# sahaRatul/sela

Hardware: AMD Instinct MI355X
Metric: Msamples/s encode+decode, 16-bit stereo 44.1kHz, 1/2/4/8 GPU; bit-exact vs CPU (higher is better)
Workload: dtype f64+int64

## Files before the change

### include/sela_hip_debug.h

```cpp
#ifndef SELA_HIP_DEBUG_H_
#define SELA_HIP_DEBUG_H_

#include <stddef.h>
#include <stdint.h>

#ifdef __cplusplus
extern "C" {
#endif

void sela_hip_debug_phase_buffer(uint64_t* d_cycles);
void sela_hip_debug_force_plain_fir(int enable);
void sela_hip_debug_mean_workers(int self_blocks);
void sela_hip_debug_encode_teams(int lanes);
int sela_hip_debug_encode_kernel(uint32_t n_frames, uint32_t channels);
void sela_hip_debug_encode_fused(int enable);
void sela_hip_debug_priorities(uint32_t team_quarters);
void sela_hip_debug_priorities_adaptive(void);
int sela_hip_debug_launches_alone(void);
void sela_hip_debug_keep_both_candidates(int on);
void sela_hip_debug_stage_wait(int naps);
int sela_hip_debug_reissued_feeds(void);
void sela_hip_debug_decode_recurrence(int form);
int sela_hip_debug_contexts_created(void);
void sela_hip_debug_coalesced(int kind, long long* batches, long long* retried);
size_t sela_hip_debug_verify_lds_bytes(uint32_t channels);
size_t sela_hip_debug_levels_lds_bytes(uint32_t channels);
size_t sela_hip_debug_digest_lds_bytes(uint32_t channels);
long long sela_hip_debug_verify_i32_fallback_frames(const void* d_workspace, uint32_t max_frames, uint32_t channels, uint32_t stride);
long long sela_hip_debug_verify_pcm_fallback_frames(const void* d_workspace, uint32_t max_frames, uint32_t channels, uint32_t stride);
long long sela_hip_debug_levels_i32_fallback_frames(const void* d_workspace, uint32_t max_frames, uint32_t channels, uint32_t stride);
long long sela_hip_debug_digest_pcm_fallback_frames(const void* d_workspace, uint32_t max_frames, uint32_t channels, uint32_t stride);

void sela_hip_debug_encode_hashes(int on);
int sela_hip_debug_block_forms(const void* d_workspace, uint32_t n_frames, uint32_t channels, uint32_t* counts_out, uint8_t* forms_out);
void sela_hip_debug_encode_split(int mode);
int sela_hip_debug_launches_split(void);
void sela_hip_debug_standard_first(int mode);
int sela_hip_debug_standard_chunks(void);
long long sela_hip_debug_segment_subframes(void);
void sela_hip_debug_generic_wrap_taps(int on);
size_t sela_hip_debug_window_lds_bytes(uint32_t channels);
uint64_t sela_hip_debug_windows_staged_bytes(void);
enum {
    SELA_HIP_WORKSPACE_ENCODE = 0, SELA_HIP_WORKSPACE_DECODE, SELA_HIP_WORKSPACE_INDEX, SELA_HIP_WORKSPACE_DECODE_I32, SELA_HIP_WORKSPACE_DECODE_N,
    SELA_HIP_WORKSPACE_VERIFY, SELA_HIP_WORKSPACE_VERIFY_I32, SELA_HIP_WORKSPACE_ENCODE_I32, SELA_HIP_WORKSPACE_ENCODE_PAIRED, SELA_HIP_WORKSPACE_WINDOWS,
// ... 11 lines not shown
```

### sela_amd/capi.py

```python
from __future__ import annotations

import ctypes as C
import os

HERE = os.path.dirname(os.path.abspath(__file__))
LIB_PATH = os.path.join(HERE, "libsela_hip.so")

OK = 0
ERRORS = {-1: "ENODEV", -2: "EINVAL", -3: "ENOMEM", -4: "ECAPACITY", -5: "EFORMAT", -6: "ERANGE"}
SAMPLES_PER_FRAME = 2048

FLAG_Q_RANGE, FLAG_COEF_OVERFLOW, FLAG_RICE_RANGE, FLAG_RICE_OVERRUN, FLAG_WORDS_CAP, FLAG_BAD_FRAME, FLAG_INTERNAL, FLAG_SHORT_BLOCK = 1, 2, 4, 8, 16, 32, 64, 128
FLAG_STRIDE = 256

EXPORTS = [
    "sela_hip_init", "sela_hip_shutdown", "sela_hip_thread_release", "sela_hip_last_error", "sela_hip_device_count",
    "sela_hip_signals_per_frame", "sela_hip_encode_workspace_bytes", "sela_hip_decode_workspace_bytes",
    "sela_hip_encode_bound_bytes", "sela_hip_encode_device", "sela_hip_decode_device",
    "sela_hip_encode", "sela_hip_decode", "sela_hip_index_frames",
    "sela_hip_enable_kernel_timing", "sela_hip_kernel_times",
    "sela_hip_lpc_encode", "sela_hip_lpc_decode", "sela_hip_rice_encode", "sela_hip_rice_decode",
    "sela_hip_host_alloc", "sela_hip_host_free", "sela_hip_decode_max_channels",
    "sela_hip_encode_begin", "sela_hip_encode_feed", "sela_hip_encode_end",
    "sela_hip_decode_begin", "sela_hip_decode_feed", "sela_hip_decode_end",
# ... 22 lines not shown
    "sela_hip_encode_pcm_device", "sela_hip_decode_pcm_workspace_bytes", "sela_hip_decode_pcm_device", "sela_hip_decode_pcm_status_error",
    "sela_hip_encode_pcm", "sela_hip_decode_pcm",
    "sela_hip_verify_pcm_workspace_bytes", "sela_hip_verify_pcm_device", "sela_hip_verify_payload_pcm_device", "sela_hip_verify_pcm",
    "sela_hip_levels_workspace_bytes", "sela_hip_levels_device", "sela_hip_levels_payload_device", "sela_hip_levels",
    "sela_hip_levels_i32_workspace_bytes", "sela_hip_levels_i32_device", "sela_hip_levels_payload_i32_device", "sela_hip_levels_samples_i32_workspace_bytes",
    "sela_hip_levels_samples_i32_device", "sela_hip_levels_i32",
    "sela_hip_digest_workspace_bytes", "sela_hip_digest_device", "sela_hip_digest_payload_device", "sela_hip_digest", "sela_hip_crc32_combine",
    "sela_hip_crc32_workspace_bytes", "sela_hip_crc32_device",
    "sela_hip_digest_pcm_workspace_bytes", "sela_hip_digest_pcm_device", "sela_hip_digest_payload_pcm_device", "sela_hip_digest_pcm",
    "sela_hip_salvage_frames", "sela_hip_salvage_workspace_bytes", "sela_hip_salvage_frames_device", "sela_hip_salvage_payload_device",
]
WINDOW_I16_INTERLEAVED, WINDOW_F32_PLANAR = 0, 1
WINDOW_I32_PLANAR, WINDOW_PCM24_INTERLEAVED, WINDOW_PCM32_INTERLEAVED = 2, 3, 4
ENCODE_LOSSLESS = 1



DEBUG_EXPORTS = [
    "sela_hip_debug_phase_buffer", "sela_hip_debug_force_plain_fir", "sela_hip_debug_mean_workers", "sela_hip_debug_encode_teams", "sela_hip_debug_encode_kernel", "sela_hip_debug_encode_fused", "sela_hip_debug_priorities", "sela_hip_debug_priorities_adaptive", "sela_hip_debug_launches_alone", "sela_hip_debug_block_forms", "sela_hip_debug_encode_hashes", "sela_hip_debug_standard_first", "sela_hip_debug_standard_chunks", "sela_hip_debug_segment_subframes", "sela_hip_debug_generic_wrap_taps", "sela_hip_debug_encode_split", "sela_hip_debug_launches_split", "sela_hip_debug_keep_both_candidates", "sela_hip_debug_stage_wait",
    "sela_hip_debug_reissued_feeds", "sela_hip_debug_contexts_created", "sela_hip_debug_decode_recurrence", "sela_hip_debug_coalesced", "sela_hip_debug_verify_lds_bytes",
    "sela_hip_debug_verify_i32_fallback_frames", "sela_hip_debug_window_lds_bytes", "sela_hip_debug_windows_staged_bytes",
    "sela_hip_debug_workspace_pieces", "sela_hip_debug_pcm_chunk_frames", "sela_hip_debug_verify_pcm_fallback_frames",
    "sela_hip_debug_levels_lds_bytes", "sela_hip_debug_levels_i32_fallback_frames", "sela_hip_debug_digest_lds_bytes",
    "sela_hip_debug_digest_pcm_fallback_frames",
]
WORKSPACE_CALLS = ("encode", "decode", "index", "decode_i32", "decode_n", "verify", "verify_i32", "encode_i32", "encode_paired", "windows", "windows_whole",
                   "encode_whole", "encode_split", "decode_whole", "windows_i32", "windows_i32_whole", "encode_whole_pcm", "salvage")


class Trace(C.Structure):
    _fields_ = [
        ("mean", C.c_double), ("ac", C.c_double * 101), ("k", C.c_double * 100), ("a", C.c_int64 * 101),
        ("q", C.c_int32 * 100), ("order", C.c_int32), ("coef_k", C.c_uint32), ("coef_words", C.c_uint32),
        ("res_k", C.c_uint32), ("res_words", C.c_uint32), ("flags", C.c_uint32),
    ]


class SelaHipError(RuntimeError):
    def __init__(self, code: int, message: str):
        super().__init__(f"libsela_hip: {ERRORS.get(code, code)}: {message}")
        self.code = code


_LIB = None


def lib() -> C.CDLL:
# ... 274 lines not shown
    L.sela_hip_debug_standard_first.restype = None
    L.sela_hip_debug_standard_chunks.argtypes = []
    L.sela_hip_debug_standard_chunks.restype = C.c_int
    L.sela_hip_debug_segment_subframes.argtypes = []
    L.sela_hip_debug_segment_subframes.restype = C.c_longlong
    L.sela_hip_debug_generic_wrap_taps.argtypes = [C.c_int]
    L.sela_hip_debug_generic_wrap_taps.restype = None
    L.sela_hip_debug_encode_split.argtypes = [C.c_int]
    L.sela_hip_debug_encode_split.restype = None
    L.sela_hip_debug_launches_split.argtypes = []
    L.sela_hip_debug_launches_split.restype = C.c_int
    L.sela_hip_debug_block_forms.argtypes = [C.c_void_p, C.c_uint32, C.c_uint32, C.c_void_p, C.c_void_p]
    L.sela_hip_debug_block_forms.restype = C.c_int
    L.sela_hip_debug_keep_both_candidates.argtypes = [C.c_int]
    L.sela_hip_debug_keep_both_candidates.restype = None
    L.sela_hip_debug_encode_kernel.argtypes = [C.c_uint32, C.c_uint32]
    L.sela_hip_debug_encode_kernel.restype = C.c_int
    L.sela_hip_debug_stage_wait.argtypes = [C.c_int]
    L.sela_hip_debug_stage_wait.restype = None
    L.sela_hip_debug_reissued_feeds.argtypes = []
    L.sela_hip_debug_reissued_feeds.restype = C.c_int
    L.sela_hip_debug_decode_recurrence.argtypes = [C.c_int]
    L.sela_hip_debug_decode_recurrence.restype = None
    L.sela_hip_debug_contexts_created.argtypes = []
    L.sela_hip_debug_contexts_created.restype = C.c_int
    L.sela_hip_debug_coalesced.argtypes = [C.c_int, C.POINTER(C.c_longlong), C.POINTER(C.c_longlong)]
    L.sela_hip_debug_coalesced.restype = None
    L.sela_hip_debug_verify_lds_bytes.argtypes = [u32]
    L.sela_hip_debug_verify_lds_bytes.restype = sz
    L.sela_hip_debug_verify_i32_fallback_frames.argtypes = [vp, u32, u32, u32]
    L.sela_hip_debug_verify_pcm_fallback_frames.argtypes = [vp, u32, u32, u32]
    L.sela_hip_debug_verify_pcm_fallback_frames.restype = C.c_longlong
    L.sela_hip_debug_verify_i32_fallback_frames.restype = C.c_longlong
    L.sela_hip_debug_window_lds_bytes.argtypes = [u32]
    L.sela_hip_debug_window_lds_bytes.restype = sz
    L.sela_hip_debug_windows_staged_bytes.argtypes = []
    L.sela_hip_debug_windows_staged_bytes.restype = C.c_uint64
    L.sela_hip_debug_workspace_pieces.argtypes = [C.c_int, u64, u32, u32, u64p, C.c_int]
    L.sela_hip_debug_workspace_pieces.restype = C.c_int
    L.sela_hip_host_alloc.argtypes = [sz]
    L.sela_hip_host_alloc.restype = C.c_void_p
    L.sela_hip_host_free.argtypes = [C.c_void_p]
    L.sela_hip_host_free.restype = None
    L.sela_hip_decode_max_channels.argtypes = []
    L.sela_hip_decode_max_channels.restype = u32
    L.sela_hip_encode_begin.argtypes = [C.POINTER(C.c_void_p), u32, u32, vp, sz, vp]
# ... 32 lines not shown
```

### sela_amd/csrc/sela_capi.hip

```cpp
#include <hip/hip_runtime.h>

#include <algorithm>
#include <atomic>

#include <chrono>
#include <condition_variable>
#include <deque>
#include <thread>
#include <cstdio>
#include <cstdlib>
#include <cstring>
#include <map>
#include <mutex>
#include <string>
#include <vector>

#include "sela_coalescer.h"
#include "sela_crc32.h"
#include "sela_decode_whole_plan.h"
#include "sela_host.h"
#include "sela_lease.h"
#include "sela_pcm.h"
#include "sela_salvage_walk.h"

// ... 53 lines not shown
    for (const Verdict& v : table)
        if ((flags & v.flag) && (v.routes & route))
            return fail(v.code, v.named ? std::string(who) + ": " + v.text : std::string(v.text));
    return SELA_HIP_OK;
}

}
namespace sela {
int report_error(int code, const std::string& what) { return fail(code, what); }
int report_hip_error(hipError_t e, const char* where) { return fail_hip(e, where); }
int device_ready()
{
    int n = 0;
    if (hipGetDeviceCount(&n) != hipSuccess || n <= 0)
        return fail(SELA_HIP_ENODEV, "no HIP device visible (the SELA MI355X path has no CPU fallback)");
    return SELA_HIP_OK;
}
int check_frame_offsets(const uint64_t* frame_offsets, uint32_t n_frames)
{
    return frame_offsets_ascend(frame_offsets, n_frames) ? SELA_HIP_OK : fail(SELA_HIP_EFORMAT, "frame offsets must not decrease");
}
int judge_decode(uint32_t flags, uint32_t judged, DecodeRoute route, const char* who) { return judge(kDecodeVerdicts, flags & judged, 1u << route, who); }
int judge_encode(uint32_t flags, uint32_t judged, const char* who) { return judge(kEncodeVerdicts, flags & judged, kEveryRoute, who); }
}
namespace {

struct PinnedPool {
    struct Block {
        void* ptr;
        size_t cap;
        bool pinned;
    };
    std::mutex mu;
    std::vector<Block> live, idle;
    size_t idle_bytes = 0;
    static constexpr size_t kIdleCap = (size_t)1 << 30;

    void* take(size_t bytes)
    {
        std::lock_guard<std::mutex> lock(mu);
        size_t best = idle.size();
        for (size_t i = 0; i < idle.size(); i++)
            if (idle[i].cap >= bytes && idle[i].cap <= 2 * bytes + 4096 && (best == idle.size() || idle[i].cap < idle[best].cap))
                best = i;
        Block b;
        if (best != idle.size()) {
// ... 1060 lines not shown
        }
    }
    if (e != hipSuccess)
        return fail_hip(e, "block forms");
    for (size_t b = 0; b < blocks; b++) {
        const uint32_t form = (meta[b].flags & sela::kBlockFormPlain) ? 2 : ((meta[b].flags & sela::kBlockFormTwoPass) ? 1 : 0);
        counts_out[form]++;
        if (forms_out)
            forms_out[b] = (uint8_t)form;
    }
    return SELA_HIP_OK;
}
void sela_hip_debug_keep_both_candidates(int on) { sela::set_keep_both_candidates(on); }
void sela_hip_debug_encode_split(int mode) { g_encode_split.store(mode < 0 || mode > 999 ? 0 : mode, std::memory_order_relaxed); }
int sela_hip_debug_launches_split(void) { return g_launches_split.load(std::memory_order_relaxed); }
void sela_hip_debug_encode_hashes(int on) { sela::set_encode_hashes(on); }
int sela_hip_debug_encode_kernel(uint32_t n_frames, uint32_t channels) { return sela::encode_team_lanes(n_frames, channels, g_team_lanes); }

void sela_hip_debug_stage_wait(int naps) { g_stage_wait_naps = naps; }

int sela_hip_debug_reissued_feeds(void) { return g_reissued_feeds; }
void sela_hip_debug_decode_recurrence(int form) { g_recurrence_form = form < 0 ? -1 : (form != 0); }
int sela_hip_debug_contexts_created(void) { return g_contexts_created.load(std::memory_order_relaxed); }

void sela_hip_enable_kernel_timing(int enable) { g_timing.enabled = enable != 0; }

int sela_hip_kernel_times(float* ms_out, int capacity)
{
    const int n = g_timing.recorded < capacity ? g_timing.recorded : capacity;
    for (int i = 0; i < n; i++) {
        if (hipEventSynchronize(g_timing.ev[i + 1]) != hipSuccess || hipEventElapsedTime(&ms_out[i], g_timing.ev[i], g_timing.ev[i + 1]) != hipSuccess)
            return 0;
    }
    return n;
}

uint32_t sela_hip_signals_per_frame(uint32_t channels) { return channels == 2 ? 3u : channels; }

size_t sela_hip_encode_workspace_bytes(uint32_t n_frames, uint32_t channels)
{
    const size_t whole = sela::encode_workspace_bytes(n_frames, channels);
    return sela::encode_split_frames(n_frames, channels, 500) ? whole + sela::encode_workspace_bytes(0, channels) + 65536 : whole;
}

size_t sela_hip_decode_workspace_bytes(uint32_t n_frames, uint32_t channels) { return sela::decode_workspace_bytes(n_frames, channels); }

// ... 2265 lines not shown
```

### sela_amd/csrc/sela_decode_core.inc

```

constexpr int kDecMaxWaves = 8;
constexpr int kDecMaxChannels = 255;
constexpr int kCoefLanes = 4;
constexpr int kResLanes = kWave - kCoefLanes;
constexpr int kStreamCap = 1072;
constexpr int kStreamMargin = 4;
constexpr uint32_t kEndOfStream = 0xFFFFFFFFu;

typedef uint32_t u32x4 __attribute__((ext_vector_type(4)));

struct SynthTables {
    union {
        int64_t a[104];
        uint64_t tab[192];
    };
};
struct DecWaveScratch {
    SynthTables t;
};
constexpr int kCoefValuesAt = 896;
static_assert(kCoefValuesAt + 104 * 4 <= (int)sizeof(SynthTables) && kCoefValuesAt >= 104 * 8, "the coefficient values lie behind a[] inside the table's space");
__device__ __forceinline__ int32_t* coef_values(DecWaveScratch* s)
{
    return reinterpret_cast<int32_t*>(reinterpret_cast<unsigned char*>(&s->t) + kCoefValuesAt);
}
union DecSubframeLds {
    uint32_t marks[kStreamCap + kStreamMargin];
    uint16_t pos[kBlock];
    int16_t smp[kBlock];
};
static_assert(sizeof(DecSubframeLds) == (kStreamCap + kStreamMargin) * 4 && sizeof(DecSubframeLds) % 16 == 0, "LDS plan");
static_assert(32 * (kStreamCap + kStreamMargin) <= 65536, "positions are 16-bit");

__device__ __forceinline__ void analyse4(__amdgpu_buffer_rsrc_t rs, uint32_t p, uint32_t k, uint32_t (&off)[5], bool& simple)
{
    const uint32_t b = 4 * (p >> 5), sh = p & 31;
    const u32x4 w = __builtin_amdgcn_raw_buffer_load_b128(rs, b, 0, 0);
    const uint32_t w4 = __builtin_amdgcn_raw_buffer_load_b32(rs, b + 16, 0, 0);
    uint32_t n0 = __builtin_amdgcn_alignbit(w.y, w.x, sh), n1 = __builtin_amdgcn_alignbit(w.z, w.y, sh);
    uint32_t n2 = __builtin_amdgcn_alignbit(w.w, w.z, sh), n3 = __builtin_amdgcn_alignbit(w4, w.w, sh);
    uint32_t used = 0;
    simple = true;
#pragma unroll
    for (int j = 0; j < 4; j++) {
        const uint32_t t = (uint32_t)__builtin_ctz(~n0 | 0x80000000u);
        const uint32_t len = t + 1 + k;
        simple = simple && len <= 31;
        off[j] = used;
        used += len;
        if (j < 3) {
            n0 = __builtin_amdgcn_alignbit(n1, n0, len);
            n1 = __builtin_amdgcn_alignbit(n2, n1, len);
            if (j < 2)
                n2 = __builtin_amdgcn_alignbit(n3, n2, len);
            if (j < 1)
                n3 >>= len & 31;
        }
    }
    off[4] = used;
}

__device__ __forceinline__ void single_step(__amdgpu_buffer_rsrc_t rs, uint32_t p, uint32_t k, uint32_t& adv, bool& full)
{
    const uint32_t b = 4 * (p >> 5), sh = p & 31;
    const uint32_t x = __builtin_amdgcn_alignbit(__builtin_amdgcn_raw_buffer_load_b32(rs, b + 4, 0, 0), __builtin_amdgcn_raw_buffer_load_b32(rs, b, 0, 0), sh);
    full = x == 0xFFFFFFFFu;
    adv = full ? 32u : (uint32_t)__builtin_ctz(~x | 0x80000000u) + 1 + k;
}

struct ParseProfile {
    long long t[4];
};

__device__ __forceinline__ int32_t decode_at(__amdgpu_buffer_rsrc_t rs, uint32_t p, uint32_t k, uint32_t kmask, bool valid)
{
    uint32_t x0, x1, ones = 0;
    window64(rs, p, x0, x1);
    while (__any(valid && x0 == 0xFFFFFFFFu)) {
        const bool more = valid && x0 == 0xFFFFFFFFu;
        ones += more ? 32u : 0u;
        p += more ? 32u : 0u;
        window64(rs, p, x0, x1);
    }
    const uint32_t t = (uint32_t)__builtin_ctz(~x0 | 0x80000000u);
    const uint32_t field = (uint32_t)(((((uint64_t)x1) << 32) | x0) >> (t + 1)) & kmask;
    return rice_value(ones + t, field, k);
}

template <bool kProf>
__device__ __forceinline__ uint32_t parse_subframe(const StreamWords& sw, uint32_t* marks, uint16_t* pos_out, uint16_t* cpos, int32_t* q,
    uint32_t cw, uint32_t rw, uint32_t ck, uint32_t rk, uint32_t order, int lane, ParseProfile& prof,
    const uint32_t n_values = (uint32_t)kBlock )
{
    const __amdgpu_buffer_rsrc_t rs = stream_rsrc(sw);
    const bool coef_lane = lane < kCoefLanes;
    const uint32_t zc = max(1u, (cw + 1 + kCoefLanes - 1) / kCoefLanes);
    const uint32_t zr = max(1u, (rw + kResLanes - 1) / kResLanes);
    const uint32_t rs_word = cw + 2;
    const uint32_t last_mark_word = cw + 2 + rw + kStreamMargin - 1;
    uint32_t first_word, end_word, stream_end, k, need;
    if (coef_lane) {
        first_word = min((uint32_t)lane * zc, cw + 1);
        end_word = min((uint32_t)(lane + 1) * zc, cw + 1);
        stream_end = 24 + 32 * cw;
        k = ck;
        need = order;
    } else {
        const uint32_t r = (uint32_t)(lane - kCoefLanes);
        first_word = rs_word + min(r * zr, rw);
        end_word = rs_word + min((r + 1) * zr, rw);
        stream_end = 32 * (rs_word + rw);
        k = rk;
        need = n_values;
    }
    const uint32_t entry = lane == 0 ? 24u : 32 * first_word;
// ... 110 lines not shown
        const uint32_t zmax = max(zc, zr);
        for (uint32_t j = 0; j < zmax; j++) {
            const bool valid = on_chain && we + j < end_word;
            if (!__any(valid))
                break;
            uint32_t word = valid ? marks[we + j] : 0u;
            if (j == 0)
                word &= 0xFFFFFFFFu << (e_true & 31);
            count += (uint32_t)__builtin_popcount(word);
        }
        count = on_chain ? count + n_cont : 0u;
    }
    uint32_t idx = wave_exclusive_scan(count, lane);
    const uint32_t coef_total = (uint32_t)__builtin_amdgcn_readlane((int)idx, kCoefLanes);
    const uint32_t all_total = (uint32_t)__builtin_amdgcn_readlane((int)(idx + count), kWave - 1);
    const uint32_t res_total = all_total - coef_total;
    if (!coef_lane)
        idx -= coef_total;
    uint32_t remaining = idx < need ? min(count, need - idx) : 0u;
    wave_sync();
    if (kProf)
        prof.t[2] = clock64();

    uint16_t* out = (coef_lane ? cpos : pos_out) + idx;
    pos = on_chain ? e_true : 0u;
    in_run = false;
    bool overrun = false;
    while (__any(remaining != 0)) {
        const bool act = remaining != 0;
        uint32_t off[5];
        bool simple;
        analyse4(rs, pos, k, off, simple);
        if (!__any(act && (in_run || !simple))) {
            uint32_t adv = 0;
#pragma unroll
            for (int j = 0; j < 4; j++) {
                const bool a = (uint32_t)j < remaining;
                if (a)
                    out[j] = (uint16_t)(pos + off[j]);
                adv = a ? off[j + 1] : adv;
            }
            const uint32_t take = min(remaining, 4u);
            out += take;
            remaining -= take;
            pos += adv;
            overrun |= act && pos > stream_end;
        } else {
            uint32_t adv;
            bool full;
            single_step(rs, pos, k, adv, full);
            const bool start = act && !in_run;
            if (start)
                *out = (uint16_t)pos;
            out += start ? 1 : 0;
            pos += act ? adv : 0u;
            in_run = act ? full : in_run;
            remaining -= (act && !full) ? 1u : 0u;
            overrun |= act && !full && pos > stream_end;
        }
    }
    {
        const uint32_t listed = min(res_total, n_values), upto = min((n_values + (uint32_t)kWave - 1) & ~((uint32_t)kWave - 1), (uint32_t)kBlock);
        if (listed < upto)
            for (uint32_t i = listed + lane; i < upto; i += kWave)
                pos_out[i] = (uint16_t)(32 * (rs_word + rw + 1));
    }
    wave_sync();
    {
        const uint32_t ckmask = ck ? (0xFFFFFFFFu >> (32 - ck)) : 0u;
        for (uint32_t i0 = 0; i0 < order; i0 += kWave) {
            const uint32_t i = i0 + (uint32_t)lane;
            const bool valid = i < min(order, coef_total);
            const int32_t v = decode_at(rs, valid ? cpos[i] : 0u, ck, ckmask, valid);
            if (i < order)
                q[i] = valid ? v : 0;
        }
    }
    const bool bad = __any(overrun) || coef_total < order || res_total < n_values;
    wave_sync();
    if (kProf)
        prof.t[3] = clock64();
    return bad ? (uint32_t)SELA_HIP_FLAG_RICE_OVERRUN : 0u;
}

__device__ inline uint32_t parse_stream_serial(const uint32_t* __restrict__ words, uint32_t first_bit, uint32_t stream_end,
    uint32_t n_frame_words, uint32_t k, uint32_t count, int32_t* out, int lane)
{
    auto word_at = [&](uint32_t w) -> uint32_t { return (w < n_frame_words && 32 * w < stream_end) ? words[w] : 0u; };
    auto bit_at = [&](uint32_t p) -> uint32_t { return p < stream_end ? (word_at(p >> 5) >> (p & 31)) & 1u : 0u; };
    uint32_t pos = first_bit;
#pragma unroll 1
    for (uint32_t i = 0; i < count; i++) {
        uint32_t ones = 0;
        for (;;) {
            const uint32_t sh = pos & 31, have = 32 - sh;
            const uint32_t lo = word_at(pos >> 5) >> sh;
            const uint32_t t = (uint32_t)__builtin_ctzll(~(uint64_t)lo | ((uint64_t)1 << have));
            ones += t;
            pos += t;
            if (t < have || pos >= stream_end)
// ... 44 lines not shown
        cur.index++;
    }
    cur.ok = h.ok;
    return h;
}

__device__ inline SubHeader walk_headers(const uint8_t* fb, uint64_t fbytes, uint32_t c)
{
    HeaderCursor cur = frame_cursor(fb, fbytes);
    return walk_to(fb, fbytes, cur, c);
}

__device__ inline bool block_header_ok(const SubHeader& h, uint32_t channels)
{
    return h.ok && sela_subframe_decodable(&h) && h.n == (uint32_t)kBlock && h.channel < channels && h.type <= 1 && (h.type == 0 || h.parent < channels);
}

__device__ __forceinline__ bool predictor_table(uint32_t order, int32_t q_lo, int32_t q_hi, SynthTables* t, int lane, uint32_t& flags)
{
    step_up_from_q(order, q_lo, q_hi, t->a, lane, flags);
    return build_synth_table(t->a, t->tab, (int)order, lane);
}

template <bool kProf>
__device__ __forceinline__ void decode_subframe(const uint8_t* fb, uint64_t fbytes, const SubHeader& hd, bool fast, DecSubframeLds* sl, DecWaveScratch* scratch,
    int32_t* ws_residues, size_t ws_block, bool vec_shift, uint32_t synth_priorities , int lane, uint32_t& flags,
    long long* stamp )
{
    const uint32_t nw = hd.cw + 2 + hd.rw;
    const uint32_t* const gw = reinterpret_cast<const uint32_t*>(fb + hd.p + 4);
    const int32_t* ws_c = nullptr;
    ParseProfile pp;
    if (fast) {
        for (uint32_t w = lane; w < nw + kStreamMargin; w += kWave)
            sl->marks[w] = 0;
        wave_sync();
        if (kProf)
            stamp[2] = clock64();
        const StreamWords sw = { gw, nw };
        flags |= parse_subframe<kProf>(sw, sl->marks, sl->pos, reinterpret_cast<uint16_t*>(&scratch->t), coef_values(scratch), hd.cw, hd.rw, hd.ck, hd.rk,
            hd.order, lane, pp);
    } else {
        if (kProf)
            stamp[2] = clock64();
        int32_t* const wres = ws_residues + ws_block * kBlock;
        const uint32_t n_frame_words = (uint32_t)((fbytes - hd.p - 4) / 4);
        flags |= parse_stream_serial(gw, 24, 24 + 32 * hd.cw, n_frame_words, hd.ck, hd.order, coef_values(scratch), lane);
        flags |= parse_stream_serial(gw, 32 * (hd.cw + 2), 32 * (hd.cw + 2 + hd.rw), n_frame_words, hd.rk, (uint32_t)kBlock, wres, lane);
        asm volatile("s_waitcnt vmcnt(0)" ::: "memory");
        __builtin_amdgcn_fence(__ATOMIC_ACQUIRE, "agent");
        ws_c = wres;
        pp.t[0] = pp.t[1] = pp.t[2] = pp.t[3] = kProf ? clock64() : 0;
    }
    if (kProf)
        stamp[3] = pp.t[0], stamp[4] = pp.t[1], stamp[5] = pp.t[2], stamp[6] = pp.t[3];

    const uint32_t order = hd.order;
    const int32_t q_lo = (uint32_t)lane < order ? coef_values(scratch)[lane] : 0, q_hi = (uint32_t)lane + 64 < order ? coef_values(scratch)[lane + 64] : 0;
    wave_sync();
    const bool fits24 = predictor_table(order, q_lo, q_hi, &scratch->t, lane, flags);
    if (kProf)
        stamp[7] = clock64();
    if (synth_priorities)
        set_wave_priority((int)((synth_priorities >> (order <= 48 ? 0 : (order <= 60 ? 8 : 16))) & 0xFF));
    if (vec_shift)
        synthesize_by_order<true>(order, gw, nw, hd.rk, sl->pos, ws_c, scratch->t.tab, fits24, lane);
    else
        synthesize_by_order<false>(order, gw, nw, hd.rk, sl->pos, ws_c, scratch->t.tab, fits24, lane);
    if (synth_priorities)
        __builtin_amdgcn_s_setprio(0);
    if (kProf)
        stamp[8] = clock64();
}

constexpr uint32_t kNoSubframe = 0xFFFFFFFFu;
__device__ __forceinline__ uint32_t sub_info_word(uint32_t type, uint32_t parent, uint32_t position) { return type | (parent << 8) | (position << 16); }
__device__ __forceinline__ uint32_t sub_info_type(uint32_t info) { return info & 0xFF; }
__device__ __forceinline__ uint32_t sub_info_parent(uint32_t info) { return (info >> 8) & 0xFF; }
__device__ __forceinline__ uint32_t sub_info_position(uint32_t info) { return info >> 16; }

__host__ __device__ inline size_t decode_lds_bytes_for(uint32_t channels, int n_waves)
{
    return (size_t)channels * sizeof(DecSubframeLds) + (size_t)n_waves * sizeof(DecWaveScratch) + (size_t)channels * 4 + (size_t)n_waves * 4;
}
struct DecFrameLds {
    DecSubframeLds* sub;
    DecWaveScratch* scratch0;
    uint32_t* sub_info;
// ... 95 lines not shown
```

### sela_amd/csrc/sela_digest.hip

```cpp
#include "sela_host.h"

#include "sela_crc32_lanes.h"
#include "sela_synth.h"

namespace sela {

#include "sela_decode_core.inc"

static_assert(kVerifyFusedChannels == (uint32_t)kDecMaxWaves, "the fused route takes what k_decode_frames takes");
static_assert(sizeof(struct sela_hip_digest) == 8 && alignof(struct sela_hip_digest) == 4, "the record of include/sela_hip.h");
static_assert(offsetof(struct sela_hip_digest, crc32) == 0 && offsetof(struct sela_hip_digest, samples) == 4, "a record leaves as one 8-byte word");

constexpr uint32_t fused_piece_samples(uint32_t channels) { return channels <= 2 ? 4u : 1u; }
constexpr DigestShape fused_shape(uint32_t channels)
{
    const uint32_t g = fused_piece_samples(channels);
    return digest_shape(2 * channels * g, 64 * (channels < (uint32_t)kDecMaxWaves ? channels : (uint32_t)kDecMaxWaves), (uint32_t)kBlock / g);
}
constexpr DigestShape kFusedShapes[kDecMaxWaves + 1] = { DigestShape{}, fused_shape(1), fused_shape(2), fused_shape(3), fused_shape(4), fused_shape(5), fused_shape(6),
    fused_shape(7), fused_shape(8) };
static_assert(kFusedShapes[2].pad == 0 && kFusedShapes[2].steps == 4 && kFusedShapes[3].pad == 11 * 192 - 2048, "pieces and threads");

__global__ __launch_bounds__(kDecMaxWaves * 64) __attribute__((amdgpu_waves_per_eu(7, 8))) void k_digest_frames(const uint8_t* __restrict__ frames,
    const uint64_t* __restrict__ frame_offsets, uint32_t n_frames, uint32_t channels, struct sela_hip_digest* __restrict__ digests ,
// ... 6 lines not shown
    const int wave = __builtin_amdgcn_readfirstlane((int)(threadIdx.x / 64)), lane = threadIdx.x % 64;
    const DecFrameLds l = carve_frame_lds(dyn, channels, n_waves);

    const uint32_t f = blockIdx.x;
    if (f >= n_frames || (n_frames_found && f >= *n_frames_found))
        return;
    const bool vec_shift = f >= vec_shift_from;
    const uint8_t* const fb = frames + frame_offsets[f];
    const uint64_t fbytes = frame_offsets[f + 1] - frame_offsets[f];
    uint32_t flags = 0;
    SubHeader hd;
    bool ok;
    const bool fast = frame_prologue(l, fb, fbytes, channels, n_waves, wave, lane, hd, ok);

    for (uint32_t c = wave; c < channels; c += n_waves) {
        if (c != (uint32_t)wave) {
            hd = walk_headers(fb, fbytes, c);
            ok = block_header_ok(hd, channels);
        }
        if (!ok) {
            flags |= SELA_HIP_FLAG_BAD_FRAME;
            continue;
        }
        decode_subframe<false>(fb, fbytes, hd, fast, l.sub + c, l.scratch0 + wave, ws_residues, (size_t)f * channels + c, vec_shift, synth_priorities, lane, flags, nullptr);
        if (lane == 0)
            l.sub_info[hd.channel] = sub_info_word(hd.type, hd.parent, c);
    }
    __syncthreads();

    uint32_t r = 0;
    if (channels == 2) {
        const StereoPass sp = stereo_pass(l.sub, l.sub_info);
        for (uint32_t i4 = threadIdx.x, j = 0; i4 < (uint32_t)kBlock / 4; i4 += blockDim.x, j++) {
            const uint4 w = stereo_words(sp, i4);
            if (j)
                r = crc_mul(r, shape.stride);
            r = crc_step32(crc_step32(crc_step32(crc_step32(r, w.x), w.y), w.z), w.w);
        }
    } else if (channels == 1) {
        for (uint32_t i4 = threadIdx.x, j = 0; i4 < (uint32_t)kBlock / 4; i4 += blockDim.x, j++) {
            uint32_t v[4];
#pragma unroll
            for (uint32_t k = 0; k < 4; k++)
                v[k] = channel_value16(l.sub, l.sub_info, 0, 4 * i4 + k);
            if (j)
                r = crc_mul(r, shape.stride);
            r = crc_step32(crc_step32(r, v[0] | (v[1] << 16)), v[2] | (v[3] << 16));
// ... 274 lines not shown
```

### sela_amd/csrc/sela_synth.h

```cpp
#ifndef SELA_SYNTH_H_
#define SELA_SYNTH_H_

#include "sela_device.h"

namespace sela {

typedef const volatile __attribute__((address_space(3))) uint64_t* LdsTable;

__device__ __forceinline__ int32_t rice_value(uint32_t ones, uint32_t field, uint32_t k)
{
    const uint32_t rem = k ? (__brev(field) >> (32 - k)) : 0u;
    const uint32_t u = (ones << k) | rem;
    return (int32_t)((u >> 1) ^ (0u - (u & 1u)));
}

struct StreamWords {
    const uint32_t* words;
    uint32_t n_words;
};
__device__ __forceinline__ __amdgpu_buffer_rsrc_t stream_rsrc(const StreamWords& s)
{
    return __builtin_amdgcn_make_buffer_rsrc(
        reinterpret_cast<void*>(read_first_lane(reinterpret_cast<uint64_t>(s.words))), 0,
        4u * (uint32_t)__builtin_amdgcn_readfirstlane((int)s.n_words), 0x00020000);
}
__device__ __forceinline__ void window64(__amdgpu_buffer_rsrc_t rs, uint32_t p, uint32_t& x0, uint32_t& x1)
{
    const uint32_t b = 4 * (p >> 5), sh = p & 31;
    const uint32_t w0 = __builtin_amdgcn_raw_buffer_load_b32(rs, b, 0, 0), w1 = __builtin_amdgcn_raw_buffer_load_b32(rs, b + 4, 0, 0),
                   w2 = __builtin_amdgcn_raw_buffer_load_b32(rs, b + 8, 0, 0);
// ... 70 lines not shown
    if (kFold)
        ch -= (uint32_t)r_block << 3;
    uint32_t kept = 0;
    int32_t shifted = 0;
    if (kVecShift) {
        shifted = (int32_t)ch >> 3;
        asm volatile("" : "+v"(shifted));
    }
    __builtin_amdgcn_sched_barrier(0);
    synth_steps<R, kFold, G, kVecShift, 0>(cl, ch, ol, oh, kept, tab_lane, r_block, four, zero, pf_c, pf_o, shifted);
    s = (int32_t)((kFold ? 0u : (uint32_t)r_block) - (uint32_t)((int32_t)kept >> 3));
    return !kFold || !__any((uint32_t)(s + (1 << 23) - 1) >= (1u << 24) - 1u);
}

template <bool kOut32>
struct SynthOut {
};
template <>
struct SynthOut<true> {
    int32_t* samples;
    uint32_t n;
};

template <int R, int G, bool kVecShift, bool kOut32 = false>
__device__ __attribute__((noinline)) void synthesize(
    const uint32_t* words, uint32_t n_words, uint32_t k, uint16_t* pos_smp, const int32_t* ws,
    const uint64_t* tab, bool fold, int lane, SynthOut<kOut32> out32 = SynthOut<kOut32>())
{
    static_assert(G == 4 || G == 16, "groups are DPP banks or rows");
    const StreamWords sw = { words, n_words };
    const __amdgpu_buffer_rsrc_t rs = stream_rsrc(sw);
    k = (uint32_t)__builtin_amdgcn_readfirstlane((int)k);
    const uint32_t kmask = k ? (0xFFFFFFFFu >> (32 - k)) : 0u;
    const bool jit = read_first_lane(reinterpret_cast<uint64_t>(ws)) == 0;
    uint32_t zl[2], zh[2];
#pragma unroll
    for (int h = 0; h < 2; h++) {
        zl[h] = 0;
        zh[h] = 4;
    }
    uint32_t four = 4, zero = 0;
    asm volatile("" : "+v"(four), "+v"(zero));
    const LdsTable tab_lane = (LdsTable)(tab + lane);
    uint32_t p = 0, w0 = 0, w1 = 0, w2 = 0;
    int32_t r_ws = 0;
    uint32_t n_samples = (uint32_t)kBlock;
    if constexpr (kOut32)
        n_samples = (uint32_t)__builtin_amdgcn_readfirstlane((int)out32.n);
    const int n_blocks = kOut32 ? (int)((n_samples + 63) / 64) : kBlock / 64;
    auto issue = [&](int blk) {
        if (jit) {
            p = pos_smp[64 * blk + lane];
            const uint32_t b = 4 * (p >> 5);
            w0 = __builtin_amdgcn_raw_buffer_load_b32(rs, b, 0, 0);
            w1 = __builtin_amdgcn_raw_buffer_load_b32(rs, b + 4, 0, 0);
            w2 = __builtin_amdgcn_raw_buffer_load_b32(rs, b + 8, 0, 0);
        } else if constexpr (kOut32) {
            r_ws = (uint32_t)(64 * blk + lane) < n_samples ? ws[64 * blk + lane] : 0;
        } else {
            w2 = (uint32_t)ws[64 * blk + lane];
        }
    };
    auto land = [&]() -> int32_t {
        if (!jit)
            return kOut32 ? r_ws : (int32_t)w2;
        uint32_t x0 = __builtin_amdgcn_alignbit(w1, w0, p & 31), x1 = __builtin_amdgcn_alignbit(w2, w1, p & 31), ones = 0;
        while (__any(x0 == 0xFFFFFFFFu)) {
            const bool more = x0 == 0xFFFFFFFFu;
            ones += more ? 32u : 0u;
            p += more ? 32u : 0u;
            window64(rs, p, x0, x1);
        }
        const uint32_t t = (uint32_t)__builtin_ctz(~x0);
        const uint32_t field = (uint32_t)(((((uint64_t)x1) << 32) | x0) >> (t + 1)) & kmask;
        return rice_value(ones + t, field, k);
    };
    auto run_block = [&](int blk, uint32_t& cl, uint32_t& ch, uint32_t& ol, uint32_t& oh) {
        const int32_t r_block = land();
        if (blk + 1 < n_blocks)
            issue(blk + 1);
        int32_t s;
        bool done = false;
        fold = fold && !__any((uint32_t)(r_block + (1 << 23) - 1) >= (1u << 24) - 1u);
        if (fold) {
            const uint32_t s0 = cl, s1 = ch, s2 = ol, s3 = oh;
            done = synth_block<R, true, G, kVecShift>(r_block, s, cl, ch, ol, oh, tab_lane, four, zero);
            if (!done) {
// ... 19 lines not shown
            run_block(pair, zl[0], zh[0], zl[R - 1], zh[R - 1]);
            if (R == 2 && pair + 1 < n_blocks)
                run_block(pair + 1, zl[1], zh[1], zl[0], zh[0]);
        }
    } else {
#pragma unroll 1
        for (int blk = 0; blk < n_blocks; blk++) {
            run_block(blk, zl[0], zh[0], zl[R - 1], zh[R - 1]);
            if (R == 2) {
                const uint32_t tl = zl[0], th = zh[0];
                zl[0] = zl[1], zh[0] = zh[1];
                zl[1] = tl, zh[1] = th;
            }
        }
    }
    wave_sync();
}

template <bool kVecShift, bool kOut32 = false>
__device__ __forceinline__ void synthesize_by_order(uint32_t order, const uint32_t* words, uint32_t n_words, uint32_t k, uint16_t* pos_smp,
    const int32_t* ws, const uint64_t* tab, bool fold, int lane, SynthOut<kOut32> out32 = SynthOut<kOut32>())
{
    if (order <= 48)
        synthesize<1, 16, kVecShift, kOut32>(words, n_words, k, pos_smp, ws, tab, fold, lane, out32);
    else if (order <= 60)
        synthesize<1, 4, kVecShift, kOut32>(words, n_words, k, pos_smp, ws, tab, fold, lane, out32);
    else
        synthesize<2, 16, kVecShift, kOut32>(words, n_words, k, pos_smp, ws, tab, fold, lane, out32);
}

__device__ inline bool build_synth_table(const int64_t* a, uint64_t* tab, int order, int lane)
{
    uint64_t c[2];
    bool fits = true;
#pragma unroll
    for (int h = 0; h < 2; h++) {
        const int d = lane + 64 * h;
        const uint64_t nv = (uint64_t)(d >= 1 && d <= order ? a[d] : 0);
        const int32_t al = (int32_t)(uint32_t)nv;
        const int32_t ah = (int32_t)(uint32_t)((nv - (uint64_t)(int64_t)al) >> 32);
        fits &= ah >= -(1 << 23) && ah < (1 << 23);
        c[h] = ((uint64_t)(uint32_t)ah << 32) | (uint32_t)al;
    }
    wave_sync();
    if (order <= 60) {
        tab[lane] = c[0];
        tab[lane + 64] = c[0];
    } else {
        tab[lane] = c[0];
        tab[lane + 64] = c[1];
        tab[lane + 128] = c[0];
// ... 9 lines not shown
```

Measured before the change: 18080.

## Decode rice values during parse and feed held residues to synthesis

The parse pass now decodes the actual zigzag residue and coefficient values alongside positions and stores them as 16-bit values in the LDS position buffer. Synthesis can then read held residues straight from LDS instead of re-reading the bitstream and re-decoding each sample just in time. If any value exceeds 16 bits, the wave re-runs a position-only listing pass, counted by a new debug counter. This adds some per-symbol arithmetic to the parse loop and a fallback re-parse path.

```diff
diff --git a/include/sela_hip_debug.h b/include/sela_hip_debug.h
--- a/include/sela_hip_debug.h
+++ b/include/sela_hip_debug.h
@@ -21,6 +21,7 @@
 void sela_hip_debug_stage_wait(int naps);
 int sela_hip_debug_reissued_feeds(void);
 void sela_hip_debug_decode_recurrence(int form);
+long long sela_hip_debug_parse_redos(void);
 int sela_hip_debug_contexts_created(void);
 void sela_hip_debug_coalesced(int kind, long long* batches, long long* retried);
 size_t sela_hip_debug_verify_lds_bytes(uint32_t channels);
diff --git a/sela_amd/capi.py b/sela_amd/capi.py
--- a/sela_amd/capi.py
+++ b/sela_amd/capi.py
@@ -68,7 +68,7 @@
     "sela_hip_debug_verify_i32_fallback_frames", "sela_hip_debug_window_lds_bytes", "sela_hip_debug_windows_staged_bytes",
     "sela_hip_debug_workspace_pieces", "sela_hip_debug_pcm_chunk_frames", "sela_hip_debug_verify_pcm_fallback_frames",
     "sela_hip_debug_levels_lds_bytes", "sela_hip_debug_levels_i32_fallback_frames", "sela_hip_debug_digest_lds_bytes",
-    "sela_hip_debug_digest_pcm_fallback_frames",
+    "sela_hip_debug_digest_pcm_fallback_frames", "sela_hip_debug_parse_redos",
 ]
 WORKSPACE_CALLS = ("encode", "decode", "index", "decode_i32", "decode_n", "verify", "verify_i32", "encode_i32", "encode_paired", "windows", "windows_whole",
                    "encode_whole", "encode_split", "decode_whole", "windows_i32", "windows_i32_whole", "encode_whole_pcm", "salvage")
@@ -389,6 +389,8 @@
     L.sela_hip_debug_reissued_feeds.restype = C.c_int
     L.sela_hip_debug_decode_recurrence.argtypes = [C.c_int]
     L.sela_hip_debug_decode_recurrence.restype = None
+    L.sela_hip_debug_parse_redos.argtypes = []
+    L.sela_hip_debug_parse_redos.restype = C.c_longlong
     L.sela_hip_debug_contexts_created.argtypes = []
     L.sela_hip_debug_contexts_created.restype = C.c_int
     L.sela_hip_debug_coalesced.argtypes = [C.c_int, C.POINTER(C.c_longlong), C.POINTER(C.c_longlong)]
diff --git a/sela_amd/csrc/sela_capi.hip b/sela_amd/csrc/sela_capi.hip
--- a/sela_amd/csrc/sela_capi.hip
+++ b/sela_amd/csrc/sela_capi.hip
@@ -99,6 +99,22 @@
 }
 int judge_decode(uint32_t flags, uint32_t judged, DecodeRoute route, const char* who) { return judge(kDecodeVerdicts, flags & judged, 1u << route, who); }
 int judge_encode(uint32_t flags, uint32_t judged, const char* who) { return judge(kEncodeVerdicts, flags & judged, kEveryRoute, who); }
+
+struct ParseRedoSources {
+    long long (*take[16])();
+    int n;
+};
+static ParseRedoSources& parse_redo_sources()
+{
+    static ParseRedoSources s = { {}, 0 };
+    return s;
+}
+void parse_redo_source_add(long long (*take)())
+{
+    ParseRedoSources& s = parse_redo_sources();
+    if (s.n < 16)
+        s.take[s.n++] = take;
+}
 }
 namespace {
 
@@ -1205,6 +1221,20 @@
 int sela_hip_debug_reissued_feeds(void) { return g_reissued_feeds; }
 void sela_hip_debug_decode_recurrence(int form) { g_recurrence_form = form < 0 ? -1 : (form != 0); }
 int sela_hip_debug_contexts_created(void) { return g_contexts_created.load(std::memory_order_relaxed); }
+long long sela_hip_debug_parse_redos(void)
+{
+    if (hipDeviceSynchronize() != hipSuccess)
+        return -1;
+    long long total = 0;
+    const sela::ParseRedoSources& s = sela::parse_redo_sources();
+    for (int i = 0; i < s.n; i++) {
+        const long long n = s.take[i]();
+        if (n < 0)
+            return -1;
+        total += n;
+    }
+    return total;
+}
 
 void sela_hip_enable_kernel_timing(int enable) { g_timing.enabled = enable != 0; }
 
diff --git a/sela_amd/csrc/sela_decode_core.inc b/sela_amd/csrc/sela_decode_core.inc
--- a/sela_amd/csrc/sela_decode_core.inc
+++ b/sela_amd/csrc/sela_decode_core.inc
@@ -32,7 +32,8 @@
 static_assert(sizeof(DecSubframeLds) == (kStreamCap + kStreamMargin) * 4 && sizeof(DecSubframeLds) % 16 == 0, "LDS plan");
 static_assert(32 * (kStreamCap + kStreamMargin) <= 65536, "positions are 16-bit");
 
-__device__ __forceinline__ void analyse4(__amdgpu_buffer_rsrc_t rs, uint32_t p, uint32_t k, uint32_t (&off)[5], bool& simple)
+template <bool kVal>
+__device__ __forceinline__ void analyse4(__amdgpu_buffer_rsrc_t rs, uint32_t p, uint32_t k, uint32_t (&off)[5], bool& simple, uint32_t (&val)[4], uint32_t rshift)
 {
     const uint32_t b = 4 * (p >> 5), sh = p & 31;
     const u32x4 w = __builtin_amdgcn_raw_buffer_load_b128(rs, b, 0, 0);
@@ -46,6 +47,8 @@
         const uint32_t t = (uint32_t)__builtin_ctz(~n0 | 0x80000000u);
         const uint32_t len = t + 1 + k;
         simple = simple && len <= 31;
+        if (kVal)
+            val[j] = (t << (k & 31)) | (__brev(__builtin_amdgcn_ubfe(n0, t + 1, k)) >> rshift);
         off[j] = used;
         used += len;
         if (j < 3) {
@@ -59,6 +62,11 @@
     }
     off[4] = used;
 }
+__device__ __forceinline__ void analyse4(__amdgpu_buffer_rsrc_t rs, uint32_t p, uint32_t k, uint32_t (&off)[5], bool& simple)
+{
+    uint32_t unused[4];
+    analyse4<false>(rs, p, k, off, simple, unused, 0);
+}
 
 __device__ __forceinline__ void single_step(__amdgpu_buffer_rsrc_t rs, uint32_t p, uint32_t k, uint32_t& adv, bool& full)
 {
@@ -87,10 +95,115 @@
     return rice_value(ones + t, field, k);
 }
 
-template <bool kProf>
+template <bool kVal>
+__device__ __forceinline__ void list_pass(__amdgpu_buffer_rsrc_t rs, uint32_t k, uint16_t* out, uint32_t pos, uint32_t remaining, uint32_t stream_end,
+    bool& overrun, uint32_t& wide)
+{
+    const uint32_t kmask = k ? (0xFFFFFFFFu >> (32 - k)) : 0u, rshift = (32 - k) & 31;
+    bool in_run = false;
+    uint32_t ones = 0;
+    while (__any(remaining != 0)) {
+        const bool act = remaining != 0;
+        uint32_t off[5], u[4];
+        bool simple;
+        analyse4<kVal>(rs, pos, k, off, simple, u, rshift);
+        if (!__any(act && (in_run || !simple))) {
+            uint32_t adv = 0;
+#pragma unroll
+            for (int j = 0; j < 4; j++) {
+                const bool a = (uint32_t)j < remaining;
+                if (a) {
+                    out[j] = kVal ? (uint16_t)((u[j] >> 1) ^ (0u - (u[j] & 1u))) : (uint16_t)(pos + off[j]);
+                    if (kVal)
+                        wide |= u[j];
+                }
+                adv = a ? off[j + 1] : adv;
+            }
+            const uint32_t take = min(remaining, 4u);
+            out += take;
+            remaining -= take;
+            pos += adv;
+            overrun |= act && pos > stream_end;
+        } else if (kVal) {
+            uint32_t x0, x1;
+            window64(rs, pos, x0, x1);
+            const bool full = x0 == 0xFFFFFFFFu;
+            const uint32_t t = (uint32_t)__builtin_ctz(~x0 | 0x80000000u);
+            const uint32_t field = (uint32_t)(((((uint64_t)x1) << 32) | x0) >> (t + 1)) & kmask;
+            const uint32_t u = ((ones + t) << (k & 31)) | (__brev(field) >> rshift);
+            const bool fin = act && !full;
+            if (fin)
+                *out = (uint16_t)((u >> 1) ^ (0u - (u & 1u)));
+            wide |= fin ? u : 0u;
+            out += fin ? 1 : 0;
+            pos += act ? (full ? 32u : t + 1 + k) : 0u;
+            ones = act ? (full ? ones + 32 : 0u) : ones;
+            in_run = act ? full : in_run;
+            remaining -= fin ? 1u : 0u;
+            overrun |= fin && pos > stream_end;
+        } else {
+            uint32_t adv;
+            bool full;
+            single_step(rs, pos, k, adv, full);
+            const bool start = act && !in_run;
+            if (start)
+                *out = (uint16_t)pos;
+            out += start ? 1 : 0;
+            pos += act ? adv : 0u;
+            in_run = act ? full : in_run;
+            remaining -= (act && !full) ? 1u : 0u;
+            overrun |= act && !full && pos > stream_end;
+        }
+    }
+}
+
+__device__ __forceinline__ void coefficients_at(__amdgpu_buffer_rsrc_t rs, const uint16_t* cpos, int32_t* q, uint32_t ck, uint32_t order, uint32_t coef_total, int lane)
+{
+    const uint32_t ckmask = ck ? (0xFFFFFFFFu >> (32 - ck)) : 0u;
+    for (uint32_t i0 = 0; i0 < order; i0 += kWave) {
+        const uint32_t i = i0 + (uint32_t)lane;
+        const bool valid = i < min(order, coef_total);
+        const int32_t v = decode_at(rs, valid ? cpos[i] : 0u, ck, ckmask, valid);
+        if (i < order)
+            q[i] = valid ? v : 0;
+    }
+}
+
+static __device__ unsigned int g_parse_redos;
+void parse_redo_source_add(long long (*take)());
+static long long parse_redos_take()
+{
+    unsigned int n = 0;
+    const unsigned int zero = 0;
+    if (hipMemcpyFromSymbol(&n, HIP_SYMBOL(g_parse_redos), sizeof n) != hipSuccess || hipMemcpyToSymbol(HIP_SYMBOL(g_parse_redos), &zero, sizeof zero) != hipSuccess)
+        return -1;
+    return (long long)n;
+}
+static const struct ParseRedoSource {
+    ParseRedoSource() { parse_redo_source_add(parse_redos_take); }
+} g_parse_redo_source;
+
+__device__ __attribute__((noinline)) void relist_positions(const uint32_t* words, uint32_t n_words, uint32_t k, uint16_t* out, uint32_t pos, uint32_t remaining,
+    uint32_t stream_end, uint16_t* cpos, uint32_t ck, uint32_t order, uint32_t coef_total, int lane)
+{
+    int32_t* const q = reinterpret_cast<int32_t*>(reinterpret_cast<unsigned char*>(cpos) + kCoefValuesAt);
+    const StreamWords sw = { words, n_words };
+    const __amdgpu_buffer_rsrc_t rs = stream_rsrc(sw);
+    bool overrun = false;
+    uint32_t unused = 0;
+    if (lane == 0)
+        atomicAdd(&g_parse_redos, 1u);
+    list_pass<false>(rs, k, out, pos, remaining, stream_end, overrun, unused);
+    wave_sync();
+    coefficients_at(rs, cpos, q, (uint32_t)__builtin_amdgcn_readfirstlane((int)ck), (uint32_t)__builtin_amdgcn_readfirstlane((int)order),
+        (uint32_t)__builtin_amdgcn_readfirstlane((int)coef_total), lane);
+}
+
+template <bool kProf, bool kValues = false>
 __device__ __forceinline__ uint32_t parse_subframe(const StreamWords& sw, uint32_t* marks, uint16_t* pos_out, uint16_t* cpos, int32_t* q,
     uint32_t cw, uint32_t rw, uint32_t ck, uint32_t rk, uint32_t order, int lane, ParseProfile& prof,
-    const uint32_t n_values = (uint32_t)kBlock )
+    const uint32_t n_values = (uint32_t)kBlock ,
+    bool* listed_values = nullptr)
 {
     const __amdgpu_buffer_rsrc_t rs = stream_rsrc(sw);
     const bool coef_lane = lane < kCoefLanes;
@@ -247,60 +360,32 @@
     if (kProf)
         prof.t[2] = clock64();
 
-    uint16_t* out = (coef_lane ? cpos : pos_out) + idx;
+    uint16_t* const out = (coef_lane ? cpos : pos_out) + idx;
     pos = on_chain ? e_true : 0u;
-    in_run = false;
-    bool overrun = false;
-    while (__any(remaining != 0)) {
-        const bool act = remaining != 0;
-        uint32_t off[5];
-        bool simple;
-        analyse4(rs, pos, k, off, simple);
-        if (!__any(act && (in_run || !simple))) {
-            uint32_t adv = 0;
-#pragma unroll
-            for (int j = 0; j < 4; j++) {
-                const bool a = (uint32_t)j < remaining;
-                if (a)
-                    out[j] = (uint16_t)(pos + off[j]);
-                adv = a ? off[j + 1] : adv;
-            }
-            const uint32_t take = min(remaining, 4u);
-            out += take;
-            remaining -= take;
-            pos += adv;
-            overrun |= act && pos > stream_end;
-        } else {
-            uint32_t adv;
-            bool full;
-            single_step(rs, pos, k, adv, full);
-            const bool start = act && !in_run;
-            if (start)
-                *out = (uint16_t)pos;
-            out += start ? 1 : 0;
-            pos += act ? adv : 0u;
-            in_run = act ? full : in_run;
-            remaining -= (act && !full) ? 1u : 0u;
-            overrun |= act && !full && pos > stream_end;
-        }
-    }
+    bool overrun = false, values = false;
+    uint32_t wide = 0;
+    if (kValues) {
+        list_pass<true>(rs, k, out, pos, remaining, stream_end, overrun, wide);
+        values = !__any(wide >= 65536u);
+        if (!values)
+            relist_positions(sw.words, sw.n_words, k, out, pos, remaining, stream_end, cpos, ck, order, coef_total, lane);
+    } else
+        list_pass<false>(rs, k, out, pos, remaining, stream_end, overrun, wide);
+    if (listed_values)
+        *listed_values = values;
     {
         const uint32_t listed = min(res_total, n_values), upto = min((n_values + (uint32_t)kWave - 1) & ~((uint32_t)kWave - 1), (uint32_t)kBlock);
         if (listed < upto)
             for (uint32_t i = listed + lane; i < upto; i += kWave)
-                pos_out[i] = (uint16_t)(32 * (rs_word + rw + 1));
-    }
-    wave_sync();
-    {
-        const uint32_t ckmask = ck ? (0xFFFFFFFFu >> (32 - ck)) : 0u;
-        for (uint32_t i0 = 0; i0 < order; i0 += kWave) {
-            const uint32_t i = i0 + (uint32_t)lane;
-            const bool valid = i < min(order, coef_total);
-            const int32_t v = decode_at(rs, valid ? cpos[i] : 0u, ck, ckmask, valid);
-            if (i < order)
-                q[i] = valid ? v : 0;
-        }
-    }
+                pos_out[i] = values ? (uint16_t)0 : (uint16_t)(32 * (rs_word + rw + 1));
+    }
+    wave_sync();
+    if (kValues) {
+        if (values)
+            for (uint32_t i = (uint32_t)lane; i < order; i += kWave)
+                q[i] = i < coef_total ? (int32_t)(int16_t)cpos[i] : 0;
+    } else
+        coefficients_at(rs, cpos, q, ck, order, coef_total, lane);
     const bool bad = __any(overrun) || coef_total < order || res_total < n_values;
     wave_sync();
     if (kProf)
@@ -391,7 +476,7 @@
     return build_synth_table(t->a, t->tab, (int)order, lane);
 }
 
-template <bool kProf>
+template <bool kProf, bool kValues = true>
 __device__ __forceinline__ void decode_subframe(const uint8_t* fb, uint64_t fbytes, const SubHeader& hd, bool fast, DecSubframeLds* sl, DecWaveScratch* scratch,
     int32_t* ws_residues, size_t ws_block, bool vec_shift, uint32_t synth_priorities , int lane, uint32_t& flags,
     long long* stamp )
@@ -399,6 +484,7 @@
     const uint32_t nw = hd.cw + 2 + hd.rw;
     const uint32_t* const gw = reinterpret_cast<const uint32_t*>(fb + hd.p + 4);
     const int32_t* ws_c = nullptr;
+    bool values = false;
     ParseProfile pp;
     if (fast) {
         for (uint32_t w = lane; w < nw + kStreamMargin; w += kWave)
@@ -407,8 +493,8 @@
         if (kProf)
             stamp[2] = clock64();
         const StreamWords sw = { gw, nw };
-        flags |= parse_subframe<kProf>(sw, sl->marks, sl->pos, reinterpret_cast<uint16_t*>(&scratch->t), coef_values(scratch), hd.cw, hd.rw, hd.ck, hd.rk,
-            hd.order, lane, pp);
+        flags |= parse_subframe<kProf, kValues>(sw, sl->marks, sl->pos, reinterpret_cast<uint16_t*>(&scratch->t), coef_values(scratch), hd.cw, hd.rw, hd.ck, hd.rk,
+            hd.order, lane, pp, (uint32_t)kBlock, &values);
     } else {
         if (kProf)
             stamp[2] = clock64();
@@ -432,7 +518,12 @@
         stamp[7] = clock64();
     if (synth_priorities)
         set_wave_priority((int)((synth_priorities >> (order <= 48 ? 0 : (order <= 60 ? 8 : 16))) & 0xFF));
-    if (vec_shift)
+    if (kValues && values) {
+        if (vec_shift)
+            synthesize_held_by_order<true>(order, sl->pos, scratch->t.tab, fits24, lane);
+        else
+            synthesize_held_by_order<false>(order, sl->pos, scratch->t.tab, fits24, lane);
+    } else if (vec_shift)
         synthesize_by_order<true>(order, gw, nw, hd.rk, sl->pos, ws_c, scratch->t.tab, fits24, lane);
     else
         synthesize_by_order<false>(order, gw, nw, hd.rk, sl->pos, ws_c, scratch->t.tab, fits24, lane);
diff --git a/sela_amd/csrc/sela_digest.hip b/sela_amd/csrc/sela_digest.hip
--- a/sela_amd/csrc/sela_digest.hip
+++ b/sela_amd/csrc/sela_digest.hip
@@ -52,7 +52,7 @@
             flags |= SELA_HIP_FLAG_BAD_FRAME;
             continue;
         }
-        decode_subframe<false>(fb, fbytes, hd, fast, l.sub + c, l.scratch0 + wave, ws_residues, (size_t)f * channels + c, vec_shift, synth_priorities, lane, flags, nullptr);
+        decode_subframe<false, false>(fb, fbytes, hd, fast, l.sub + c, l.scratch0 + wave, ws_residues, (size_t)f * channels + c, vec_shift, synth_priorities, lane, flags, nullptr);
         if (lane == 0)
             l.sub_info[hd.channel] = sub_info_word(hd.type, hd.parent, c);
     }
diff --git a/sela_amd/csrc/sela_synth.h b/sela_amd/csrc/sela_synth.h
--- a/sela_amd/csrc/sela_synth.h
+++ b/sela_amd/csrc/sela_synth.h
@@ -6,6 +6,7 @@
 namespace sela {
 
 typedef const volatile __attribute__((address_space(3))) uint64_t* LdsTable;
+typedef const __attribute__((address_space(3))) int16_t* LdsResidues;
 
 __device__ __forceinline__ int32_t rice_value(uint32_t ones, uint32_t field, uint32_t k)
 {
@@ -122,17 +123,18 @@
     uint32_t n;
 };
 
-template <int R, int G, bool kVecShift, bool kOut32 = false>
+template <int R, int G, bool kVecShift, bool kHeld = false, bool kOut32 = false>
 __device__ __attribute__((noinline)) void synthesize(
     const uint32_t* words, uint32_t n_words, uint32_t k, uint16_t* pos_smp, const int32_t* ws,
     const uint64_t* tab, bool fold, int lane, SynthOut<kOut32> out32 = SynthOut<kOut32>())
 {
     static_assert(G == 4 || G == 16, "groups are DPP banks or rows");
+    static_assert(!(kHeld && kOut32), "the record holds 16-bit residues");
     const StreamWords sw = { words, n_words };
     const __amdgpu_buffer_rsrc_t rs = stream_rsrc(sw);
     k = (uint32_t)__builtin_amdgcn_readfirstlane((int)k);
     const uint32_t kmask = k ? (0xFFFFFFFFu >> (32 - k)) : 0u;
-    const bool jit = read_first_lane(reinterpret_cast<uint64_t>(ws)) == 0;
+    const bool jit = !kHeld && read_first_lane(reinterpret_cast<uint64_t>(ws)) == 0;
     uint32_t zl[2], zh[2];
 #pragma unroll
     for (int h = 0; h < 2; h++) {
@@ -149,7 +151,9 @@
         n_samples = (uint32_t)__builtin_amdgcn_readfirstlane((int)out32.n);
     const int n_blocks = kOut32 ? (int)((n_samples + 63) / 64) : kBlock / 64;
     auto issue = [&](int blk) {
-        if (jit) {
+        if constexpr (kHeld) {
+            w2 = (uint32_t)(int32_t)((LdsResidues)pos_smp)[64 * blk + lane];
+        } else if (jit) {
             p = pos_smp[64 * blk + lane];
             const uint32_t b = 4 * (p >> 5);
             w0 = __builtin_amdgcn_raw_buffer_load_b32(rs, b, 0, 0);
@@ -162,7 +166,7 @@
         }
     };
     auto land = [&]() -> int32_t {
-        if (!jit)
+        if (kHeld || !jit)
             return kOut32 ? r_ws : (int32_t)w2;
         uint32_t x0 = __builtin_amdgcn_alignbit(w1, w0, p & 31), x1 = __builtin_amdgcn_alignbit(w2, w1, p & 31), ones = 0;
         while (__any(x0 == 0xFFFFFFFFu)) {
@@ -228,11 +232,21 @@
     const int32_t* ws, const uint64_t* tab, bool fold, int lane, SynthOut<kOut32> out32 = SynthOut<kOut32>())
 {
     if (order <= 48)
-        synthesize<1, 16, kVecShift, kOut32>(words, n_words, k, pos_smp, ws, tab, fold, lane, out32);
+        synthesize<1, 16, kVecShift, false, kOut32>(words, n_words, k, pos_smp, ws, tab, fold, lane, out32);
     else if (order <= 60)
-        synthesize<1, 4, kVecShift, kOut32>(words, n_words, k, pos_smp, ws, tab, fold, lane, out32);
+        synthesize<1, 4, kVecShift, false, kOut32>(words, n_words, k, pos_smp, ws, tab, fold, lane, out32);
     else
-        synthesize<2, 16, kVecShift, kOut32>(words, n_words, k, pos_smp, ws, tab, fold, lane, out32);
+        synthesize<2, 16, kVecShift, false, kOut32>(words, n_words, k, pos_smp, ws, tab, fold, lane, out32);
+}
+template <bool kVecShift>
+__device__ __forceinline__ void synthesize_held_by_order(uint32_t order, uint16_t* pos_smp, const uint64_t* tab, bool fold, int lane)
+{
+    if (order <= 48)
+        synthesize<1, 16, kVecShift, true>(nullptr, 0, 0, pos_smp, nullptr, tab, fold, lane);
+    else if (order <= 60)
+        synthesize<1, 4, kVecShift, true>(nullptr, 0, 0, pos_smp, nullptr, tab, fold, lane);
+    else
+        synthesize<2, 16, kVecShift, true>(nullptr, 0, 0, pos_smp, nullptr, tab, fold, lane);
 }
 
 __device__ inline bool build_synth_table(const int64_t* a, uint64_t* tab, int order, int lane)
```

Result: no change. 18240 (median of 6 runs) (+0.8%).
